# colmap/glomap

Hardware: NVIDIA H100
Metric: observations/sec per BA LM-iteration (higher is better)
Workload: dtype f64

## Files before the change

glomap_b200/csrc/ba_kernels_v2.cuh:

```cuda
#pragma once
#include "ba_kernels.cuh"
#include "pcg.cuh"

namespace b200 {

struct BAViewV2 {
  const double* Ap;
  double* z4;
  const double* pts4;
  double* Ufk = nullptr;
  const IntrVarRec* ivar = nullptr;
  int C = 0;
};

template <int NK>
__device__ __forceinline__ void obs_intr_jac(const ObsCore& o, const Intr& in, const IntrVarRec& iv,
                                             double Jk[2][NK > 0 ? NK : 1]) {
#pragma unroll
  for (int j = 0; j < NK; ++j) {
    double jx = 0.0, jy = 0.0;
    if (j < iv.mb) intr_param_jac(in, iv.pidx[j], o.uv[0], o.uv[1], 1.0, jx, jy);
    if (!o.valid) jx = jy = 0.0;
    Jk[0][j] = jx;
    Jk[1][j] = jy;
  }
}
template <int NK>
__device__ __forceinline__ void obs_intr_rows(const ObsCore& o, const Intr& in, const IntrVarRec& iv,
                                              const double Jp[6], double Jk[2][NK > 0 ? NK : 1],
                                              double B[NK > 0 ? 3 * NK : 1]) {
  obs_intr_jac<NK>(o, in, iv, Jk);
#pragma unroll
  for (int j = 0; j < NK; ++j)
#pragma unroll
    for (int c = 0; c < 3; ++c) B[3 * j + c] = o.rho1 * (Jp[c] * Jk[0][j] + Jp[3 + c] * Jk[1][j]);
}

struct SegRec {
  double R[9];
  double4 t4;
  Intr in;
  const double* sr;
};
__device__ __forceinline__ void seg_records(const BAView& v, int seg, int cam, const double* __restrict__ cam_rec,
                                            const double* __restrict__ intr_rec, SegRec& s) {
  const double4 q4 = ld_rec32(cam_rec + (size_t)cam * kCamRec);
  s.t4 = ld_rec32(cam_rec + (size_t)cam * kCamRec + 4);
  s.in = ld_intr(intr_rec + (size_t)v.seg_intr[seg] * kIntrRec);
  s.sr = sensor_of_seg(v, seg);
  const double q[4] = {q4.x, q4.y, q4.z, q4.w};
  quat_to_R(q, s.R);
}
__device__ __forceinline__ void to_sensor(const double* __restrict__ sr, double x[3]) {
  if (!sr) return;
  const double x0 = x[0], x1 = x[1], x2 = x[2];
#pragma unroll
  for (int k = 0; k < 3; ++k) x[k] = sr[3 * k] * x0 + sr[3 * k + 1] * x1 + sr[3 * k + 2] * x2;
}
__device__ __forceinline__ void cam_frame_jac(const ObsCore& o, const double r[3], double a[2], double w[3]) {
  const ProjJac& p = o.pj;
  const double t0 = r[0] - p.u * r[2], t1 = r[1] - p.v * r[2];
  const double c = o.rho1 * p.iz;
  a[0] = c * (p.m00 * t0 + p.m01 * t1);
  a[1] = c * (p.m10 * t0 + p.m11 * t1);
  const double s0 = p.iz * (p.m00 * a[0] + p.m10 * a[1]), s1 = p.iz * (p.m01 * a[0] + p.m11 * a[1]);
  w[0] = s0;
  w[1] = s1;
  w[2] = -(p.u * s0 + p.v * s1);
}
__device__ __forceinline__ void rig_to_frame(const double* __restrict__ sr, double x[3]) {
  const double x0 = x[0], x1 = x[1], x2 = x[2];
#pragma unroll
  for (int k = 0; k < 3; ++k) x[k] = sr[k] * x0 + sr[3 + k] * x1 + sr[6 + k] * x2;
}
// ... 38 lines not shown
    p[i] = pv[k];
    yw[i] = 0.0;
  }
  if (c >= n_pack) return;
  const double* r = cam_rec + (size_t)c * kCamRec;
  const double q[4] = {r[0], r[1], r[2], r[3]};
  double R[9];
  quat_to_R(q, R);
  double* o = xp + (size_t)c * kXqStride;
#pragma unroll
  for (int k = 0; k < 3; ++k) {
    o[k] = R[k] * pv[0] + R[3 + k] * pv[1] + R[6 + k] * pv[2];
    o[3 + k] = R[k] * pv[3] + R[3 + k] * pv[4] + R[6 + k] * pv[5];
  }
}

__global__ void ba2_pad_points(int P, const double* __restrict__ points, double* __restrict__ pts4) {
  const int p = blockIdx.x * blockDim.x + threadIdx.x;
  if (p >= P) return;
  const double x = points[3 * (size_t)p], y = points[3 * (size_t)p + 1], z = points[3 * (size_t)p + 2];
  st_rec32(pts4 + 4 * (size_t)p, x, y, z, 0.0);
}

template <int NK>
__global__ void __launch_bounds__(128, NK > 0 ? 3 : B200_LC_MIN_CTAS) ba2_linearize_cams(BAView v, BAViewV2 v2, const double* __restrict__ cam_rec,
                                                         const double* __restrict__ intr_rec, double huber_a) {
  const int warp = (blockIdx.x * blockDim.x + threadIdx.x) >> 5;
  const int lane = threadIdx.x & 31;
  if (warp >= v.n_segs) return;
  const int cam = v.seg_cam[warp];
  const int b = v.seg_begin[warp], e = v.seg_end[warp];
  SegRec sg;
  seg_records(v, warp, cam, cam_rec, intr_rec, sg);
  double U[21], g[6];
#pragma unroll
  for (int k = 0; k < 21; ++k) U[k] = 0.0;
#pragma unroll
  for (int k = 0; k < 6; ++k) g[k] = 0.0;
  const int cmask = (int)(__double_as_longlong(sg.t4.w) & 0xff);
  const bool tvar = !(cmask & 2), rvar = !(cmask & 1);
  constexpr int NKK = NK > 0 ? NK : 1;
  const int blk = v.seg_intr[warp];
  IntrVarRec iv{};
  if (NK > 0) iv = v2.ivar[blk];
  double Ukk[NKK * (NKK + 1) / 2], gk[NKK], Ufk[6][NKK];
#pragma unroll
  for (int k = 0; k < NKK * (NKK + 1) / 2; ++k) Ukk[k] = 0.0;
#pragma unroll
  for (int k = 0; k < NKK; ++k) {
    gk[k] = 0.0;
#pragma unroll
    for (int i2 = 0; i2 < 6; ++i2) Ufk[i2][k] = 0.0;
  }
  const double* __restrict__ pts4 = v2.pts4;
  int i = b + lane;
  int pt_nxt = 0;
  double2 xy = make_double2(0, 0);
  double4 Xc = make_double4(0, 0, 0, 0);
  if (i < e) {
    const int pt0 = ld_stream(v.pt_c + i);
    if (i + 32 < e) pt_nxt = ld_stream(v.pt_c + i + 32);
    xy = ld_stream(v.xy_c + i);
    Xc = ld_rec32(pts4 + 4 * (size_t)pt0);
  }
  for (; i < e; i += 32) {
    double4 Xn = Xc;
    double2 xyn = xy;
    int pt_nn = 0;
    if (i + 32 < e) {
      Xn = ld_rec32(pts4 + 4 * (size_t)pt_nxt);
      xyn = ld_stream(v.xy_c + i + 32);
    }
    if (i + 64 < e) pt_nn = ld_stream(v.pt_c + i + 64);
    const double X0 = Xc.x, X1 = Xc.y, X2 = Xc.z;
    ObsCore o;
    obs_core_R(sg.R, sg.t4, sg.in, sg.sr, X0, X1, X2, xy, huber_a, o);
    double Jc[2][6];
#pragma unroll
    for (int a = 0; a < 2; ++a) {
      const double j0 = o.J[3 * a], j1 = o.J[3 * a + 1], j2 = o.J[3 * a + 2];
      Jc[a][0] = rvar ? -2.0 * (j1 * o.RX[2] - j2 * o.RX[1]) : 0.0;
      Jc[a][1] = rvar ? -2.0 * (j2 * o.RX[0] - j0 * o.RX[2]) : 0.0;
      Jc[a][2] = rvar ? -2.0 * (j0 * o.RX[1] - j1 * o.RX[0]) : 0.0;
      Jc[a][3] = tvar ? j0 : 0.0;
      Jc[a][4] = tvar ? j1 : 0.0;
      Jc[a][5] = tvar ? j2 : 0.0;
    }
    const double e0 = o.rho1 * o.e[0], e1 = o.rho1 * o.e[1];
    int idx = 0;
#pragma unroll
    for (int i2 = 0; i2 < 6; ++i2) {
      const double s0 = o.rho1 * Jc[0][i2], s1 = o.rho1 * Jc[1][i2];
#pragma unroll
      for (int j = i2; j < 6; ++j) U[idx++] += s0 * Jc[0][j] + s1 * Jc[1][j];
      g[i2] += Jc[0][i2] * e0 + Jc[1][i2] * e1;
    }
    if (NK > 0) {
      double Jk[2][NKK];
      obs_intr_jac<NK>(o, sg.in, iv, Jk);
      int ik = 0;
#pragma unroll
      for (int a = 0; a < NK; ++a) {
        const double s0 = o.rho1 * Jk[0][a], s1 = o.rho1 * Jk[1][a];
#pragma unroll
        for (int c = a; c < NK; ++c) Ukk[ik++] += s0 * Jk[0][c] + s1 * Jk[1][c];
        gk[a] += Jk[0][a] * e0 + Jk[1][a] * e1;
#pragma unroll
        for (int i2 = 0; i2 < 6; ++i2) Ufk[i2][a] += Jc[0][i2] * s0 + Jc[1][i2] * s1;
      }
    }
    Xc = Xn; xy = xyn; pt_nxt = pt_nn;
  }
  if (NK > 0) {
    const size_t kb = (size_t)(v2.C + blk);
    int ik = 0;
#pragma unroll
    for (int a = 0; a < NK; ++a) {
#pragma unroll
      for (int c = a; c < NK; ++c) {
        const double sacc = warp_sum(Ukk[ik++]);
        if (lane == 0 && sacc != 0.0) atomicAdd(&v.U[kb * 21 + sym_idx(6, a, c)], sacc);
      }
      const double sg = warp_sum(gk[a]);
      if (lane == 0 && sg != 0.0) atomicAdd(&v.gc[kb * 6 + a], sg);
#pragma unroll
      for (int i2 = 0; i2 < 6; ++i2) {
        const double sf = warp_sum(Ufk[i2][a]);
        if (lane == 0 && sf != 0.0) atomicAdd(&v2.Ufk[((size_t)cam * 6 + i2) * NK + a], sf);
      }
    }
  }
#pragma unroll
  for (int k = 0; k < 21; ++k) {
    const double s = warp_sum(U[k]);
    if (lane == k && s != 0.0) atomicAdd(&v.U[(size_t)cam * 21 + k], s);
  }
#pragma unroll
  for (int k = 0; k < 6; ++k) {
    const double s = warp_sum(g[k]);
    if (lane == 21 + k && s != 0.0) atomicAdd(&v.gc[(size_t)cam * 6 + k], s);
  }
}

__global__ void __launch_bounds__(128, B200_SD_MIN_CTAS) ba2_schur_diag(BAView v, BAViewV2 v2, const double* __restrict__ cam_rec,
                                                                        const double* __restrict__ intr_rec, double huber_a) {
  const int warp = (blockIdx.x * blockDim.x + threadIdx.x) >> 5;
  const int lane = threadIdx.x & 31;
  if (warp >= v.n_segs) return;
  const int cam = v.seg_cam[warp];
  const int b = v.seg_begin[warp], e = v.seg_end[warp];
  SegRec sg;
  seg_records(v, warp, cam, cam_rec, intr_rec, sg);
  double RR[6] = {0, 0, 0, 0, 0, 0}, RT[9] = {0, 0, 0, 0, 0, 0, 0, 0, 0}, TT[6] = {0, 0, 0, 0, 0, 0};
  int i = b + lane;
  int pt_nxt = 0;
  double2 xy = make_double2(0, 0), va = xy, vb = xy, vc = xy;
  double4 Xc = make_double4(0, 0, 0, 0);
  if (i < e) {
    const int pt0 = ld_stream(v.pt_c + i);
    if (i + 32 < e) pt_nxt = ld_stream(v.pt_c + i + 32);
    xy = ld_stream(v.xy_c + i);
    Xc = ld_rec32(v2.pts4 + 4 * (size_t)pt0);
    const double2* vp = reinterpret_cast<const double2*>(v.Vinv + (size_t)pt0 * 6);
    va = vp[0]; vb = vp[1]; vc = vp[2];
  }
  for (; i < e; i += 32) {
    double4 Xn = Xc;
    double2 xyn = xy, van = va, vbn = vb, vcn = vc;
    int pt_nn = 0;
    if (i + 32 < e) {
      Xn = ld_rec32(v2.pts4 + 4 * (size_t)pt_nxt);
      xyn = ld_stream(v.xy_c + i + 32);
      const double2* vp = reinterpret_cast<const double2*>(v.Vinv + (size_t)pt_nxt * 6);
      van = vp[0]; vbn = vp[1]; vcn = vp[2];
    }
    if (i + 64 < e) pt_nn = ld_stream(v.pt_c + i + 64);
    ObsCore o;
    obs_core_R(sg.R, sg.t4, sg.in, sg.sr, Xc.x, Xc.y, Xc.z, xy, huber_a, o);
    double X[3] = {o.RX[0], o.RX[1], o.RX[2]};
    to_sensor(sg.sr, X);
    const ProjJac& pj = o.pj;
    const double vi[6] = {va.x, va.y, vb.x, vb.y, vc.x, vc.y};
    double e0[3] = {1.0, 0.0, -pj.u}, e1[3] = {0.0, 1.0, -pj.v};
    if (sg.sr) {
#pragma unroll
      for (int c = 0; c < 3; ++c) {
        e0[c] = sg.sr[c] - pj.u * sg.sr[6 + c];
        e1[c] = sg.sr[3 + c] - pj.v * sg.sr[6 + c];
      }
    }
    double l0[3], l1[3], t0[3], t1[3];
#pragma unroll
    for (int c = 0; c < 3; ++c) {
      l0[c] = e0[0] * sg.R[c] + e0[1] * sg.R[3 + c] + e0[2] * sg.R[6 + c];
      l1[c] = e1[0] * sg.R[c] + e1[1] * sg.R[3 + c] + e1[2] * sg.R[6 + c];
    }
    sym3_mul(vi, l0, t0);
    sym3_mul(vi, l1, t1);
    const double q00 = l0[0] * t0[0] + l0[1] * t0[1] + l0[2] * t0[2];
    const double q01 = l0[0] * t1[0] + l0[1] * t1[1] + l0[2] * t1[2];
    const double q11 = l1[0] * t1[0] + l1[1] * t1[1] + l1[2] * t1[2];
    const double k00 = pj.m00 * pj.m00 + pj.m10 * pj.m10, k01 = pj.m00 * pj.m01 + pj.m10 * pj.m11,
                 k11 = pj.m01 * pj.m01 + pj.m11 * pj.m11;
    const double a00 = k00 * q00 + k01 * q01, a01 = k00 * q01 + k01 * q11;
    const double a10 = k01 * q00 + k11 * q01, a11 = k01 * q01 + k11 * q11;
    const double sc = o.rho1 * pj.iz * pj.iz, c2 = sc * sc;
    const double h00 = c2 * (a00 * k00 + a01 * k01), h01 = c2 * (a00 * k01 + a01 * k11), h11 = c2 * (a10 * k01 + a11 * k11);
    double N[3][3];
    N[0][0] = h00; N[0][1] = N[1][0] = h01; N[1][1] = h11;
    N[0][2] = N[2][0] = -(h00 * pj.u + h01 * pj.v);
    N[1][2] = N[2][1] = -(h01 * pj.u + h11 * pj.v);
    N[2][2] = -(N[0][2] * pj.u + N[1][2] * pj.v);
    double P[3][3];
#pragma unroll
    for (int c = 0; c < 3; ++c) {
      const double n0 = N[0][c], n1 = N[1][c], n2 = N[2][c];
      P[0][c] = 2.0 * (X[1] * n2 - X[2] * n1);
      P[1][c] = 2.0 * (X[2] * n0 - X[0] * n2);
// ... 2 lines not shown
    double PK[3][3];
#pragma unroll
    for (int r = 0; r < 3; ++r) {
      PK[r][0] = P[r][1] * X[2] - P[r][2] * X[1];
      PK[r][1] = -P[r][0] * X[2] + P[r][2] * X[0];
      PK[r][2] = P[r][0] * X[1] - P[r][1] * X[0];
    }
    RR[0] += -2.0 * PK[0][0]; RR[1] += -2.0 * PK[0][1]; RR[2] += -2.0 * PK[0][2];
    RR[3] += -2.0 * PK[1][1]; RR[4] += -2.0 * PK[1][2]; RR[5] += -2.0 * PK[2][2];
#pragma unroll
    for (int r = 0; r < 3; ++r)
#pragma unroll
      for (int c = 0; c < 3; ++c) RT[3 * r + c] += P[r][c];
    TT[0] += N[0][0]; TT[1] += N[0][1]; TT[2] += N[0][2]; TT[3] += N[1][1]; TT[4] += N[1][2]; TT[5] += N[2][2];
    Xc = Xn; xy = xyn; va = van; vb = vbn; vc = vcn; pt_nxt = pt_nn;
  }
#pragma unroll
  for (int k = 0; k < 6; ++k) RR[k] = warp_sum(RR[k]);
#pragma unroll
  for (int k = 0; k < 9; ++k) RT[k] = warp_sum(RT[k]);
#pragma unroll
  for (int k = 0; k < 6; ++k) TT[k] = warp_sum(TT[k]);
  if (lane == 0) {
    const int mask = (int)(__double_as_longlong(sg.t4.w) & 0xff);
    double R[9] = {1, 0, 0, 0, 1, 0, 0, 0, 1};
    if (sg.sr) {
      for (int r = 0; r < 3; ++r)
        for (int c = 0; c < 3; ++c) R[3 * r + c] = sg.sr[3 * c + r];
    }
    double M[6][6];
    const double rr[3][3] = {{RR[0], RR[1], RR[2]}, {RR[1], RR[3], RR[4]}, {RR[2], RR[4], RR[5]}};
    const double tt[3][3] = {{TT[0], TT[1], TT[2]}, {TT[1], TT[3], TT[4]}, {TT[2], TT[4], TT[5]}};
    for (int r = 0; r < 3; ++r)
      for (int c = 0; c < 3; ++c) {
        M[r][c] = rr[r][c];
        M[3 + r][3 + c] = tt[r][c];
        M[r][3 + c] = RT[3 * r + c];
        M[3 + c][r] = RT[3 * r + c];
      }
    double T[6][6];
    for (int blk = 0; blk < 2; ++blk)
      for (int r = 0; r < 3; ++r)
        for (int c = 0; c < 6; ++c)
          T[3 * blk + r][c] = R[3 * r] * M[3 * blk][c] + R[3 * r + 1] * M[3 * blk + 1][c] + R[3 * r + 2] * M[3 * blk + 2][c];
    int idx = 0;
    for (int r = 0; r < 6; ++r)
      for (int c = r; c < 6; ++c, ++idx) {
        const int cb = c / 3, cc = c % 3;
        double s = T[r][3 * cb] * R[3 * cc] + T[r][3 * cb + 1] * R[3 * cc + 1] + T[r][3 * cb + 2] * R[3 * cc + 2];
        const bool rfix = (r < 3) ? (mask & 1) : (mask & 2), cfix = (c < 3) ? (mask & 1) : (mask & 2);
        if (rfix || cfix) s = 0.0;
// ... 168 lines not shown
  a0 = block_sum(a0, scratch);
  a1 = block_sum(a1, scratch);
  a2 = block_sum(a2, scratch);
  a3 = block_sum(a3, scratch);
  if (threadIdx.x == 0) {
    double* o = out + 4 * (size_t)blockIdx.x;
    o[0] = a0; o[1] = a1; o[2] = a2; o[3] = a3;
  }
}

__global__ void ba2_point_rhs_z(BAView v, BAViewV2 v2) {
  const int p = blockIdx.x * blockDim.x + threadIdx.x;
  if (p >= v.P) return;
  double vi[6], g[3], z[3];
#pragma unroll
  for (int k = 0; k < 6; ++k) vi[k] = v.Vinv[6 * (size_t)p + k];
#pragma unroll
  for (int k = 0; k < 3; ++k) g[k] = v.gp[3 * (size_t)p + k];
  sym3_mul(vi, g, z);
  const bool pvalid = (int)(v.pt_begin[p + 1] - v.pt_begin[p]) >= v.min_views;
  *reinterpret_cast<double4*>(v2.z4 + 4 * (size_t)p) = pvalid ? make_double4(z[0], z[1], z[2], 0.0) : make_double4(0, 0, 0, 0);
}

template <int NK>
__global__ void __launch_bounds__(128, B200_PB_MIN_CTAS) ba2_pass_b(BAView v, BAViewV2 v2, const double* __restrict__ cam_rec,
                                                 const double* __restrict__ intr_rec, double huber_a,
                                                 double* __restrict__ y, const PcgCtl* __restrict__ ctl, int seg_lo,
                                                 int seg_hi) {
  if (ctl && ctl->done) return;
  const int warp = seg_lo + ((blockIdx.x * blockDim.x + threadIdx.x) >> 5);
  const int lane = threadIdx.x & 31;
  if (warp >= seg_hi) return;
  const int cam = v.seg_cam[warp];
  const int b = v.seg_begin[warp], e = v.seg_end[warp];
  const int blk = v.seg_intr[warp];
  SegRec sg;
  seg_records(v, warp, cam, cam_rec, intr_rec, sg);
  constexpr int NKK = NK > 0 ? NK : 1;
  IntrVarRec iv{};
  if (NK > 0) iv = v2.ivar[blk];
  double acc[6] = {0, 0, 0, 0, 0, 0};
  double accK[NKK];
#pragma unroll
  for (int k = 0; k < NKK; ++k) accK[k] = 0.0;
  const uint64_t keep = l2_policy_evict_last();
  int i = b + lane;
  int pt_nxt = 0;
  double4 X = make_double4(0, 0, 0, 0), z = X;
  double2 xy = make_double2(0, 0);
  if (i < e) {
    const int pt0 = ld_stream(v.pt_c + i);
    if (i + 32 < e) pt_nxt = ld_stream(v.pt_c + i + 32);
    X = ld_rec32(v2.pts4 + 4 * (size_t)pt0);
    z = ld_keep4(v2.z4 + 4 * (size_t)pt0, keep);
    xy = ld_stream(v.xy_c + i);
  }
  for (; i < e; i += 32) {
    double4 Xn = X, zn = z;
    double2 xyn = xy;
    int pt_nn = 0;
    if (i + 32 < e) {
      Xn = ld_rec32(v2.pts4 + 4 * (size_t)pt_nxt);
      zn = ld_keep4(v2.z4 + 4 * (size_t)pt_nxt, keep);
      xyn = ld_stream(v.xy_c + i + 32);
    }
    if (i + 64 < e) pt_nn = ld_stream(v.pt_c + i + 64);
    ObsCore o;
    obs_core_R(sg.R, sg.t4, sg.in, sg.sr, X.x, X.y, X.z, xy, huber_a, o);
    double P[3] = {o.RX[0], o.RX[1], o.RX[2]};
    to_sensor(sg.sr, P);
    double r[3] = {sg.R[0] * z.x + sg.R[1] * z.y + sg.R[2] * z.z,
                   sg.R[3] * z.x + sg.R[4] * z.y + sg.R[5] * z.z,
                   sg.R[6] * z.x + sg.R[7] * z.y + sg.R[8] * z.z};
    to_sensor(sg.sr, r);
    double a[2], w[3];
    cam_frame_jac(o, r, a, w);
    acc[0] += P[1] * w[2] - P[2] * w[1];
    acc[1] += P[2] * w[0] - P[0] * w[2];
    acc[2] += P[0] * w[1] - P[1] * w[0];
    acc[3] += w[0];
    acc[4] += w[1];
    acc[5] += w[2];
    if (NK > 0) {
      double Jk[2][NKK];
      obs_intr_jac<NK>(o, sg.in, iv, Jk);
#pragma unroll
      for (int k = 0; k < NK; ++k) accK[k] += Jk[0][k] * a[0] + Jk[1][k] * a[1];
    }
    X = Xn; z = zn; xy = xyn; pt_nxt = pt_nn;
  }
#pragma unroll
  for (int k = 0; k < 6; ++k) acc[k] = warp_sum(acc[k]);
  if (sg.sr) {
    rig_to_frame(sg.sr, acc);
    rig_to_frame(sg.sr, acc + 3);
  }
  const int mask = (int)(__double_as_longlong(sg.t4.w) & 0xff);
#pragma unroll
  for (int k = 0; k < 6; ++k) {
    const double s = k < 3 ? 2.0 * acc[k] : acc[k];
    const bool fixed = k < 3 ? (mask & 1) : (mask & 2);
    if (lane == k && !fixed && s != 0.0) atomicAdd(&y[(size_t)cam * 6 + k], -s);
  }
  if (NK > 0) {
    const size_t kb = (size_t)(v2.C + blk);
#pragma unroll
    for (int k = 0; k < NK; ++k) {
      const double sk = warp_sum(accK[k]);
      if (lane == 0 && sk != 0.0) atomicAdd(&y[kb * 6 + k], -sk);
    }
  }
}

__global__ void ba2k_pack_xk(int C, const double* __restrict__ cam_rec, const double* __restrict__ x, double* __restrict__ xp,
                             const PcgCtl* __restrict__ ctl) {
  if (ctl && ctl->done) return;
  const int c = blockIdx.x * blockDim.x + threadIdx.x;
  if (c >= C) return;
  const int blk = (int)(__double_as_longlong(cam_rec[(size_t)c * kCamRec + 7]) >> 8);
  xp[(size_t)c * kXqStride + 6] = x[(size_t)(C + blk) * 6];
// ... 54 lines not shown
```

glomap_b200/csrc/ba_solver.cuh:

```cuda
#pragma once
#include <cub/cub.cuh>

#include <algorithm>
#include <climits>
#include <cmath>
#include <cstdlib>
#include <vector>

#include "../../include/b200sfm_testing.h"
#include "ba_kernels.cuh"
#include "ba_kernels_v2.cuh"
#include "ba_kernels_v3.cuh"
#include "ba_kernels_ext.cuh"
#include "filter_kernels.cuh"
#include "processor_kernels.cuh"
#include "context.cuh"
#include "pcg.cuh"

namespace b200 {

constexpr double kSliceL2Share = 1.0 / 6.0;

__global__ void k_expand_obs_pt(int P, const unsigned* __restrict__ pt_begin, int* __restrict__ obs_pt) {
  const int p = blockIdx.x * blockDim.x + threadIdx.x;
// ... 125 lines not shown
  b200::ExtView ext_view() {
    b200::ExtView e;
    e.C = C; e.K = K; e.S = S; e.ivar = ivar.p; e.sensor_var = (ext_s && S > 0) ? sensor_var.p : nullptr;
    return e;
  }
  bool use_v2 = false;
  bool use_ell = false;
  int ell_groups = 0, ell_ctas = 0, ell_bpart_rows = 0;
  long long ell_rows = 0;
  DevBuf<int> ell_row0, ell_pt, ell_len, ell_slot, ell_cam;
  DevBuf<double2> ell_xy;
  DevBuf<unsigned short> ell_sensor;
  DevBuf<double> ell_A, ell_part;
  b200::EllView ell_view() {
    b200::EllView e;
    e.n_groups = ell_groups; e.row0 = ell_row0.p; e.pt = ell_pt.p; e.len = ell_len.p; e.cam = ell_cam.p; e.xy = ell_xy.p;
    e.sensor = S > 0 ? ell_sensor.p : nullptr; e.A = ell_A.p; e.B = kfast ? ell_B.p : nullptr;
    return e;
  }
  DevBuf<double> z4, pts4, xq, bpart, bpart2;
  size_t smem_k3v2 = 0;
  bool kfast = false;
  int nk = 0;
  DevBuf<double> ell_B, Ufk;
  b200::BAViewV2 view2() {
    b200::BAViewV2 w;
    w.Ap = W.p; w.z4 = z4.p; w.pts4 = pts4.p;
    w.Ufk = kfast ? Ufk.p : nullptr; w.ivar = ivar.p; w.C = C;
    return w;
  }
  int cur = 0;
  DevBuf<double> cam_rec, intr_rec;
  DevBuf<double> W, V, Vinv, gp, lin , Sd, Minv, jscale_c, jscale_p, Dc;
  DevBuf<double> px, pr, pz, pp, pq, yw, bvec;
  DevBuf<double> scal;
  b200::EventTimer timer_lin, timer_mv;
  size_t smem_k1 = 0, smem_k3 = 0;

  double* U() { return lin.p; }
  double* gc() { return lin.p + (size_t)CB * 21; }
  double* cost_ptr() { return lin.p + (size_t)CB * 27; }

  BAView view() {
    BAView v;
    v.C = C; v.P = P; v.K = K; v.N = N; v.n_tiles = n_tiles; v.n_segs = n_segs; v.min_views = min_views;
    v.obs_cam = obs_cam.p; v.obs_pt = obs_pt.p; v.obs_xy = obs_xy.p; v.pt_begin = pt_begin.p;
// ... 335 lines not shown
    }
    if (use_ell) {
      const int nwp = ell_ctas * (kEllThreads / 32);
#define B200_LIN_P(NKV)                                                                                                   \
  B200_LAUNCH(ctx, ba3_linearize_points<NKV>, ell_ctas, kEllThreads, 0, v, ell_view(), cam_rec.p, intr_rec.p, points[cur].p, \
              huber_a, points_var ? 1 : 0, ell_part.p, ell_part.p + nwp, ivar.p)
      if (kfast && nk == 2) B200_LIN_P(2);
      else if (kfast && nk == 1) B200_LIN_P(1);
      else B200_LIN_P(0);
#undef B200_LIN_P
      B200_LAUNCH(ctx, ba3_reduce_partials, 1, 1024, 0, nwp, ell_part.p, ell_part.p + nwp, scal.p, scal.p + 1);
    } else if (use_v2)
      B200_LAUNCH(ctx, ba_linearize_points<true>, n_tiles, kTile, smem_k1, v, cam_rec.p, intr_rec.p, points[cur].p, huber_a,
                  points_var ? 1 : 0, scal.p);
    else
      B200_LAUNCH(ctx, ba_linearize_points<false>, n_tiles, kTile, smem_k1, v, cam_rec.p, intr_rec.p, points[cur].p, huber_a,
                  points_var ? 1 : 0, scal.p);
    if (profile) B200_CUDA_OK(cudaEventRecord(e1, s));
    if (n_segs > 0) {
      const int sgrid = cdiv((long long)n_segs * 32, 128);
      if (kfast) {
        Ufk.zero(s);
        B200_LAUNCH(ctx, ba2_pad_points, cdiv(P, 256), 256, 0, P, points[cur].p, pts4.p);
        if (nk == 2) B200_LAUNCH(ctx, ba2_linearize_cams<2>, sgrid, 128, 0, v, view2(), cam_rec.p, intr_rec.p, huber_a);
        else B200_LAUNCH(ctx, ba2_linearize_cams<1>, sgrid, 128, 0, v, view2(), cam_rec.p, intr_rec.p, huber_a);
      } else if (ext) {
        B200_LAUNCH(ctx, bax_linearize_blocks<0>, sgrid, 128, 0, v, ext_view(), cam_rec.p, intr_rec.p, points[cur].p, huber_a);
        if (ext_k) B200_LAUNCH(ctx, bax_linearize_blocks<1>, sgrid, 128, 0, v, ext_view(), cam_rec.p, intr_rec.p, points[cur].p, huber_a);
        if (ext_s) B200_LAUNCH(ctx, bax_linearize_blocks<2>, sgrid, 128, 0, v, ext_view(), cam_rec.p, intr_rec.p, points[cur].p, huber_a);
      } else if (use_v2) {
        B200_LAUNCH(ctx, ba2_pad_points, cdiv(P, 256), 256, 0, P, points[cur].p, pts4.p);
        B200_LAUNCH(ctx, ba2_linearize_cams<0>, sgrid, 128, 0, v, view2(), cam_rec.p, intr_rec.p, huber_a);
      } else {
        B200_LAUNCH(ctx, ba_linearize_cams, sgrid, 128, 0, v, cam_rec.p, intr_rec.p, points[cur].p, huber_a);
      }
    }
    B200_CUDA_OK(cudaMemcpyAsync(cost_ptr(), scal.p, sizeof(double), cudaMemcpyDeviceToDevice, s));
    B200_CUDA_OK(cudaMemcpyAsync(cost_ptr() + 1 + ctx->rank, scal.p + 1, sizeof(double), cudaMemcpyDeviceToDevice, s));
    ctx->allreduce_sum(lin.p, (size_t)CB * 27 + 1 + (size_t)ctx->world);
    B200_CUDA_OK(cudaMemsetAsync(scal.p + 1, 0, sizeof(double), s));
    B200_LAUNCH(ctx, ba_finalize_cams, cdiv(nbk, 128), 128, 0, nbk, U(), gc(), cam_mask.p, jscale_c.p, first ? 1 : 0,
                scal.p, cost_ptr() + 1, ctx->world);
    B200_CUDA_OK(cudaMemcpyAsync(ctx->h_scal, cost_ptr(), sizeof(double), cudaMemcpyDeviceToHost, s));
    B200_CUDA_OK(cudaMemcpyAsync(ctx->h_scal + 1, scal.p + 1, sizeof(double), cudaMemcpyDeviceToHost, s));
    B200_CUDA_OK(cudaStreamSynchronize(s));
    cost = ctx->h_scal[0];
    gmax = ctx->h_scal[1];
  }

  DevBuf<double> bear_res;
  void undistort(double* h_out) {
    using namespace b200;
    cudaStream_t s = ctx->stream;
    if (bear_res.n < (size_t)N * 3) bear_res.alloc((size_t)std::max<long long>(N, 1) * 3);
    if (N > 0)
// ... 117 lines not shown
      if (ext_k && ext_s) B200_EXT_A(true, true);
      else if (ext_k) B200_EXT_A(true, false);
      else if (ext_s) B200_EXT_A(false, true);
      else B200_EXT_A(false, false);
#undef B200_EXT_A
    }
    if (n_segs > 0) {
#define B200_EXT_B(WK, WS)                                                                                              \
  B200_LAUNCH(ctx, (bax_pass_b<WK, WS>), sgrid, 128, 0, v, ex, view2(), cam_rec.p, intr_rec.p, points[cur].p, x, huber_a, y, ctl)
      if (ext_k && ext_s) B200_EXT_B(true, true);
      else if (ext_k) B200_EXT_B(true, false);
      else if (ext_s) B200_EXT_B(false, true);
      else B200_EXT_B(false, false);
#undef B200_EXT_B
    }
  }

  void launch_pass_b(const b200::BAView& v, double huber_a, double* y, const b200::PcgCtl* ctl, int seg_lo = 0,
                     int seg_hi = -1) {
    using namespace b200;
    if (seg_hi < 0) seg_hi = n_segs;
    if (seg_hi <= seg_lo) return;
    const int grid = cdiv((long long)(seg_hi - seg_lo) * 32, 128);
#define B200_PASS_B(NKV) \
  B200_LAUNCH(ctx, ba2_pass_b<NKV>, grid, 128, 0, v, view2(), cam_rec.p, intr_rec.p, huber_a, y, ctl, seg_lo, seg_hi)
    if (kfast && nk == 2) B200_PASS_B(2);
    else if (kfast) B200_PASS_B(1);
    else B200_PASS_B(0);
#undef B200_PASS_B
  }
  void launch_pass_a0(const b200::BAView& v, double radius, const b200::PcgCtl* ctl) {
    using namespace b200;
    if (kfast && nk == 2)
      B200_LAUNCH(ctx, (ba3_pass_a<0, 2>), ell_ctas, kEllThreads, 0, v, ell_view(), view2(), xq.p, points[cur].p, nullptr, radius, nullptr, ctl);
    else if (kfast)
      B200_LAUNCH(ctx, (ba3_pass_a<0, 1>), ell_ctas, kEllThreads, 0, v, ell_view(), view2(), xq.p, points[cur].p, nullptr, radius, nullptr, ctl);
    else
      B200_LAUNCH(ctx, (ba3_pass_a<0, 0>), ell_ctas, kEllThreads, 0, v, ell_view(), view2(), xq.p, points[cur].p, nullptr, radius, nullptr, ctl);
  }
  void launch_cross(const double* x, double* y, const b200::PcgCtl* ctl) {
    using namespace b200;
    if (nk == 2) B200_LAUNCH(ctx, ba2k_cross<2>, cdiv(C, 256), 256, 0, C, K, cam_rec.p, Ufk.p, x, y, ctl);
    else B200_LAUNCH(ctx, ba2k_cross<1>, cdiv(C, 256), 256, 0, C, K, cam_rec.p, Ufk.p, x, y, ctl);
  }

  bool matrix_free() const { return ext && !kfast; }
  bool schur_jacobi_on(const b200sfm_ba_opts& o, bool points_var) const {
    return points_var && o.preconditioner == 1 && !matrix_free();
  }

  void matvec(const double* x, double* y, const b200sfm_ba_opts& o, double radius, bool points_var, bool split_ar,
// ... 33 lines not shown
                  nullptr, 0, ctl);
    }
    if (profile) B200_CUDA_OK(cudaEventRecord(e1, s));
    if (split_ar) {
      ctx->allreduce_sum(y + (size_t)(C / 2) * 6, nB6 - (size_t)(C / 2) * 6);
      B200_CUDA_OK(cudaStreamWaitEvent(s, ctx->ev_comm, 0));
    } else {
      ctx->allreduce_sum(y, nB6);
    }
  }

  StepResult compute_step(const b200sfm_ba_opts& o, double radius, bool points_var, bool set_jscale_p, bool profile) {
    using namespace b200;
    cudaStream_t s = ctx->stream;
    BAView v = view();
    const int nB6 = nbk * 6;
    if (points_var) B200_LAUNCH(ctx, ba_damp_points, cdiv(P, 256), 256, 0, P, V.p, jscale_p.p, set_jscale_p ? 1 : 0, radius, Vinv.p);
    B200_LAUNCH(ctx, ba_damp_cams, cdiv(nB6, 256), 256, 0, nbk, U(), jscale_c.p, radius, Dc.p);
    const bool recomp = matrix_free();
    const bool schur_jacobi = schur_jacobi_on(o, points_var);
    double* yrhs = Sd.p + (size_t)CB * 21;
    Sd.zero(s);
    if (schur_jacobi && n_segs > 0) {
      if (use_v2)
        B200_LAUNCH(ctx, ba2_schur_diag, cdiv((long long)n_segs * 32, 128), 128, 0, v, view2(), cam_rec.p, intr_rec.p,
                    o.thres_loss_function);
      else B200_LAUNCH(ctx, ba_schur_diag, cdiv((long long)n_segs * 32, 128), 128, 0, v);
    }
    if (points_var) {
      if (use_v2) {
        B200_LAUNCH(ctx, ba2_point_rhs_z, cdiv(P, 256), 256, 0, v, view2());
        if (recomp) ext_matvec(nullptr, yrhs, o.thres_loss_function, radius, true, nullptr);
        else if (n_segs > 0) launch_pass_b(v, o.thres_loss_function, yrhs, nullptr);
      } else {
        B200_LAUNCH(ctx, ba_schur_pass<1>, n_tiles, kTile, smem_k3, v, nullptr, yrhs, nullptr, nullptr, radius, nullptr);
      }
    } else if (recomp) {
      z4.zero(s);
    }
    if (schur_jacobi || points_var) ctx->allreduce_sum(Sd.p, (size_t)CB * 27);
    B200_LAUNCH(ctx, ba_build_precond, cdiv(nbk, 128), 128, 0, nbk, U(), Dc.p, schur_jacobi ? Sd.p : nullptr, Minv.p);
    B200_LAUNCH(ctx, k_rhs, cdiv(nB6, 256), 256, 0, nB6, gc(), points_var ? yrhs : nullptr, bvec.p);
    const int max_it = std::max(1, o.pcg_max_iterations);
    const int nblk = cdiv(nbk, kPcgThreads);
    ctx->pcgh.ensure(max_it, (size_t)nblk * 3, ctx->world);
    double* part_pq = ctx->pcgh.d_part;
    double* part_rz = ctx->pcgh.d_part + nblk;
    double* part_rr = ctx->pcgh.d_part + 2 * (size_t)nblk;
    PcgCtl* ctl = ctx->pcgh.d_ctl;
    StepResult res;
// ... 111 lines not shown
          for (int j = 0; j < 3; ++j)
            if (nfoc[h_intr_model[k]][j] >= 0) idx.push_back(nfoc[h_intr_model[k]][j]);
        if (all_var) { idx.push_back(pp[h_intr_model[k]][0]); idx.push_back(pp[h_intr_model[k]][1]); }
        std::sort(idx.begin(), idx.end());
        h_ivar[k].col0 = 0;
        h_ivar[k].mb = (int)idx.size();
        for (size_t j = 0; j < idx.size(); ++j) h_ivar[k].pidx[j] = idx[j];
        ext_k = ext_k || !idx.empty();
      }
      B200_CUDA_OK(cudaMemcpyAsync(ivar.p, h_ivar.data(), K * sizeof(b200::IntrVarRec), cudaMemcpyHostToDevice, s));
    }
    ext_s = false;
    if (o.optimize_rig_poses && S > 0)
      for (int i = 0; i < S; ++i) ext_s = ext_s || h_sensor_var[i] != 0;
    ext = ext_k || ext_s;
    nbk = ext ? CB : C;
    B200_CUDA_OK(cudaStreamSynchronize(s));
    use_v2 = ext || (o.design != 1);
    use_ell = use_v2 && (ext || !(getenv("B200SFM_ELL") && atoi(getenv("B200SFM_ELL")) == 0));
    nk = 0;
    if (ext_k)
      for (int k = 0; k < K; ++k) nk = std::max(nk, h_ivar[k].mb);
    kfast = ext_k && !ext_s && S == 0 && nk <= 2 && !(getenv("B200SFM_KFAST") && atoi(getenv("B200SFM_KFAST")) == 0);
    if (kfast) {
      const size_t cells = (size_t)std::max<long long>(ell_rows, 1) * 32;
      if (ell_B.n < cells * 3 * nk) ell_B.alloc(cells * 3 * nk);
      if (Ufk.n < (size_t)C * 6 * nk) Ufk.alloc((size_t)C * 6 * nk);
    }
  }
  void launch_eff_mask(const b200sfm_ba_opts& o) {
    B200_LAUNCH(ctx, b200::k_eff_mask, b200::cdiv(C, 256), 256, 0, C, cam_mask_base.p, o.optimize_rotations ? 0 : 1,
                o.optimize_translation ? 0 : 1, cam_mask.p);
  }

  void reject_step() { build_records(cur); }

  int solve(const b200sfm_ba_opts& o, b200sfm_lm_stats* st) {
    using namespace b200;
    cudaStream_t s = ctx->stream;
    select_paths(o);
    const bool l2_persist = use_v2 && !(getenv("B200SFM_L2_PERSIST") && atoi(getenv("B200SFM_L2_PERSIST")) == 0) &&
                            l2_persist_window(s, ctx->device, z4.p, z4.bytes());
    const long long launches0 = ctx->launches;
    timer_lin.reset();
    timer_mv.reset();
    cudaEvent_t ev0, ev1;
// ... 159 lines not shown
```

glomap_b200/csrc/common.cuh:

```cuda
#pragma once
#include <cuda_runtime.h>
#include <stdint.h>
#include <stdio.h>

#include <string>

namespace b200 {

#ifndef B200_TILE
#define B200_TILE 128
#endif
#ifndef B200_K1_MIN_CTAS
#define B200_K1_MIN_CTAS 5
#endif
#ifndef B200_K3_MIN_CTAS
#define B200_K3_MIN_CTAS 8
#endif
#ifndef B200_PA_MIN_CTAS
#define B200_PA_MIN_CTAS 12
#endif
#ifndef B200_LC_MIN_CTAS
#define B200_LC_MIN_CTAS 3
#endif
#ifndef B200_PB_MIN_CTAS
#define B200_PB_MIN_CTAS 4
#endif
#ifndef B200_SD_MIN_CTAS
#define B200_SD_MIN_CTAS 3
#endif
#ifndef B200_E1_MIN_CTAS
#define B200_E1_MIN_CTAS 4
#endif
#ifndef B200_E1_PIPE
#define B200_E1_PIPE 1
#endif
#ifndef B200_EA_MIN_CTAS
#define B200_EA_MIN_CTAS 8
#endif
#ifndef B200_EA2_MIN_CTAS
#define B200_EA2_MIN_CTAS 6
#endif
#ifndef B200_STREAM_HINTS
#define B200_STREAM_HINTS 1
#endif
constexpr int kTile = B200_TILE;
constexpr int kTilePts = 64;
constexpr int kWDoubles = 18;
constexpr int kWBytes = kWDoubles * 8;

#define B200_CUDA_OK(expr)                                                                     \
  do {                                                                                         \
// ... 275 lines not shown
```

Baseline: 1.573 billion.

## Stage per-segment camera records in shared memory and specialize kernels on radial/rig

Per-segment camera rotation, translation, intrinsics and sensor transform move out of per-thread registers into a 256-byte shared-memory record per warp. Each observation reloads them with explicit ld.shared. The kernels gain compile-time RAD/RIG template flags, so the non-radial and non-rig variants drop the distortion and sensor-transform code, and the host picks the variant at launch. The point is to lower register pressure so more CTAs fit per SM, and minimum-CTA launch bounds go from 3 to 4 for the linearize and Schur-diagonal kernels. The cost is extra shared-memory loads in the inner loop and the risk of register spills under the tighter bounds.

```diff
diff --git a/glomap_b200/csrc/ba_kernels_v2.cuh b/glomap_b200/csrc/ba_kernels_v2.cuh
--- a/glomap_b200/csrc/ba_kernels_v2.cuh
+++ b/glomap_b200/csrc/ba_kernels_v2.cuh
@@ -36,20 +36,59 @@
     for (int c = 0; c < 3; ++c) B[3 * j + c] = o.rho1 * (Jp[c] * Jk[0][j] + Jp[3 + c] * Jk[1][j]);
 }
 
-struct SegRec {
+struct SegSmem {
+  double R[9], t[3];
+  double fx, fy, cx, cy, k1, k2, model;
+  double packed;
+  double sr[12];
+};
+static_assert(sizeof(SegSmem) == 32 * sizeof(double), "one 256-B record per warp");
+template <bool RIG>
+__device__ __forceinline__ void seg_fill(const BAView& v, int seg, int cam, const double* __restrict__ cam_rec,
+                                         const double* __restrict__ intr_rec, SegSmem& s) {
+  const double4 q4 = ld_rec32(cam_rec + (size_t)cam * kCamRec);
+  const double4 t4 = ld_rec32(cam_rec + (size_t)cam * kCamRec + 4);
+  const double q[4] = {q4.x, q4.y, q4.z, q4.w};
   double R[9];
-  double4 t4;
-  Intr in;
-  const double* sr;
-};
-__device__ __forceinline__ void seg_records(const BAView& v, int seg, int cam, const double* __restrict__ cam_rec,
-                                            const double* __restrict__ intr_rec, SegRec& s) {
-  const double4 q4 = ld_rec32(cam_rec + (size_t)cam * kCamRec);
-  s.t4 = ld_rec32(cam_rec + (size_t)cam * kCamRec + 4);
-  s.in = ld_intr(intr_rec + (size_t)v.seg_intr[seg] * kIntrRec);
-  s.sr = sensor_of_seg(v, seg);
-  const double q[4] = {q4.x, q4.y, q4.z, q4.w};
-  quat_to_R(q, s.R);
+  quat_to_R(q, R);
+#pragma unroll
+  for (int k = 0; k < 9; ++k) s.R[k] = R[k];
+  s.t[0] = t4.x; s.t[1] = t4.y; s.t[2] = t4.z;
+  s.packed = t4.w;
+  const double* ir = intr_rec + (size_t)v.seg_intr[seg] * kIntrRec;
+  s.fx = ir[0]; s.fy = ir[1]; s.cx = ir[2]; s.cy = ir[3]; s.k1 = ir[4]; s.k2 = ir[5]; s.model = ir[6];
+  if (RIG) {
+    const double* sr = v.sensor_rec + (size_t)v.seg_sensor[seg] * kSensorRec;
+#pragma unroll
+    for (int k = 0; k < 12; ++k) s.sr[k] = sr[k];
+  }
+}
+__device__ __forceinline__ double lds(const double* p) {
+  double x;
+  asm volatile("ld.shared.f64 %0, [%1];" : "=d"(x) : "r"((unsigned)__cvta_generic_to_shared(p)) : "memory");
+  return x;
+}
+__device__ __forceinline__ void seg_R(const SegSmem& s, double R[9]) {
+#pragma unroll
+  for (int k = 0; k < 9; ++k) R[k] = lds(&s.R[k]);
+}
+__device__ __forceinline__ double4 seg_t4(const SegSmem& s) { return make_double4(lds(&s.t[0]), lds(&s.t[1]), lds(&s.t[2]), 0.0); }
+template <int N>
+__device__ __forceinline__ void seg_sensor(const SegSmem& s, double sr[12]) {
+#pragma unroll
+  for (int k = 0; k < N; ++k) sr[k] = lds(&s.sr[k]);
+}
+template <int NK, bool RAD>
+__device__ __forceinline__ Intr seg_intr(const SegSmem& s) {
+  return Intr{lds(&s.fx), lds(&s.fy), lds(&s.cx), lds(&s.cy), RAD ? lds(&s.k1) : 0.0, RAD ? lds(&s.k2) : 0.0,
+              NK > 0 ? (int)lds(&s.model) : 0};
+}
+template <int NK, bool RAD, bool RIG>
+__device__ __forceinline__ void seg_obs_core(const SegSmem& s, const double R[9], double X0, double X1, double X2,
+                                             double2 xy, double huber_a, ObsCore& o) {
+  double sr[12];
+  if (RIG) seg_sensor<12>(s, sr);
+  obs_core_R(R, seg_t4(s), seg_intr<NK, RAD>(s), RIG ? sr : nullptr, X0, X1, X2, xy, huber_a, o);
 }
 __device__ __forceinline__ void to_sensor(const double* __restrict__ sr, double x[3]) {
   if (!sr) return;
@@ -134,22 +173,24 @@
   st_rec32(pts4 + 4 * (size_t)p, x, y, z, 0.0);
 }
 
-template <int NK>
-__global__ void __launch_bounds__(128, NK > 0 ? 3 : B200_LC_MIN_CTAS) ba2_linearize_cams(BAView v, BAViewV2 v2, const double* __restrict__ cam_rec,
+template <int NK, bool RAD, bool RIG>
+__global__ void __launch_bounds__(128, NK > 0 ? B200_LCK_MIN_CTAS : (RIG ? B200_RIG_MIN_CTAS : B200_LC_MIN_CTAS)) ba2_linearize_cams(BAView v, BAViewV2 v2, const double* __restrict__ cam_rec,
                                                          const double* __restrict__ intr_rec, double huber_a) {
+  __shared__ SegSmem seg_sm[4];
   const int warp = (blockIdx.x * blockDim.x + threadIdx.x) >> 5;
   const int lane = threadIdx.x & 31;
   if (warp >= v.n_segs) return;
   const int cam = v.seg_cam[warp];
   const int b = v.seg_begin[warp], e = v.seg_end[warp];
-  SegRec sg;
-  seg_records(v, warp, cam, cam_rec, intr_rec, sg);
+  if (lane == 0) seg_fill<RIG>(v, warp, cam, cam_rec, intr_rec, seg_sm[threadIdx.x >> 5]);
+  __syncwarp();
+  const SegSmem& sg = seg_sm[threadIdx.x >> 5];
   double U[21], g[6];
 #pragma unroll
   for (int k = 0; k < 21; ++k) U[k] = 0.0;
 #pragma unroll
   for (int k = 0; k < 6; ++k) g[k] = 0.0;
-  const int cmask = (int)(__double_as_longlong(sg.t4.w) & 0xff);
+  const int cmask = (int)(__double_as_longlong(lds(&sg.packed)) & 0xff);
   const bool tvar = !(cmask & 2), rvar = !(cmask & 1);
   constexpr int NKK = NK > 0 ? NK : 1;
   const int blk = v.seg_intr[warp];
@@ -186,7 +227,11 @@
     if (i + 64 < e) pt_nn = ld_stream(v.pt_c + i + 64);
     const double X0 = Xc.x, X1 = Xc.y, X2 = Xc.z;
     ObsCore o;
-    obs_core_R(sg.R, sg.t4, sg.in, sg.sr, X0, X1, X2, xy, huber_a, o);
+    {
+      double R[9];
+      seg_R(sg, R);
+      seg_obs_core<NK, RAD, RIG>(sg, R, X0, X1, X2, xy, huber_a, o);
+    }
     double Jc[2][6];
 #pragma unroll
     for (int a = 0; a < 2; ++a) {
@@ -209,7 +254,7 @@
     }
     if (NK > 0) {
       double Jk[2][NKK];
-      obs_intr_jac<NK>(o, sg.in, iv, Jk);
+      obs_intr_jac<NK>(o, seg_intr<NK, RAD>(sg), iv, Jk);
       int ik = 0;
 #pragma unroll
       for (int a = 0; a < NK; ++a) {
@@ -254,15 +299,18 @@
   }
 }
 
-__global__ void __launch_bounds__(128, B200_SD_MIN_CTAS) ba2_schur_diag(BAView v, BAViewV2 v2, const double* __restrict__ cam_rec,
+template <bool RAD, bool RIG>
+__global__ void __launch_bounds__(128, RIG ? B200_RIG_MIN_CTAS : B200_SD_MIN_CTAS) ba2_schur_diag(BAView v, BAViewV2 v2, const double* __restrict__ cam_rec,
                                                                         const double* __restrict__ intr_rec, double huber_a) {
+  __shared__ SegSmem seg_sm[4];
   const int warp = (blockIdx.x * blockDim.x + threadIdx.x) >> 5;
   const int lane = threadIdx.x & 31;
   if (warp >= v.n_segs) return;
   const int cam = v.seg_cam[warp];
   const int b = v.seg_begin[warp], e = v.seg_end[warp];
-  SegRec sg;
-  seg_records(v, warp, cam, cam_rec, intr_rec, sg);
+  if (lane == 0) seg_fill<RIG>(v, warp, cam, cam_rec, intr_rec, seg_sm[threadIdx.x >> 5]);
+  __syncwarp();
+  const SegSmem& sg = seg_sm[threadIdx.x >> 5];
   double RR[6] = {0, 0, 0, 0, 0, 0}, RT[9] = {0, 0, 0, 0, 0, 0, 0, 0, 0}, TT[6] = {0, 0, 0, 0, 0, 0};
   int i = b + lane;
   int pt_nxt = 0;
@@ -288,24 +336,34 @@
     }
     if (i + 64 < e) pt_nn = ld_stream(v.pt_c + i + 64);
     ObsCore o;
-    obs_core_R(sg.R, sg.t4, sg.in, sg.sr, Xc.x, Xc.y, Xc.z, xy, huber_a, o);
+    {
+      double R[9];
+      seg_R(sg, R);
+      seg_obs_core<0, RAD, RIG>(sg, R, Xc.x, Xc.y, Xc.z, xy, huber_a, o);
+    }
     double X[3] = {o.RX[0], o.RX[1], o.RX[2]};
-    to_sensor(sg.sr, X);
     const ProjJac& pj = o.pj;
     const double vi[6] = {va.x, va.y, vb.x, vb.y, vc.x, vc.y};
     double e0[3] = {1.0, 0.0, -pj.u}, e1[3] = {0.0, 1.0, -pj.v};
-    if (sg.sr) {
+    if (RIG) {
+      double sr[12];
+      seg_sensor<9>(sg, sr);
+      to_sensor(sr, X);
 #pragma unroll
       for (int c = 0; c < 3; ++c) {
-        e0[c] = sg.sr[c] - pj.u * sg.sr[6 + c];
-        e1[c] = sg.sr[3 + c] - pj.v * sg.sr[6 + c];
+        e0[c] = sr[c] - pj.u * sr[6 + c];
+        e1[c] = sr[3 + c] - pj.v * sr[6 + c];
       }
     }
     double l0[3], l1[3], t0[3], t1[3];
-#pragma unroll
-    for (int c = 0; c < 3; ++c) {
-      l0[c] = e0[0] * sg.R[c] + e0[1] * sg.R[3 + c] + e0[2] * sg.R[6 + c];
-      l1[c] = e1[0] * sg.R[c] + e1[1] * sg.R[3 + c] + e1[2] * sg.R[6 + c];
+    {
+      double R[9];
+      seg_R(sg, R);
+#pragma unroll
+      for (int c = 0; c < 3; ++c) {
+        l0[c] = e0[0] * R[c] + e0[1] * R[3 + c] + e0[2] * R[6 + c];
+        l1[c] = e1[0] * R[c] + e1[1] * R[3 + c] + e1[2] * R[6 + c];
+      }
     }
     sym3_mul(vi, l0, t0);
     sym3_mul(vi, l1, t1);
@@ -354,11 +412,11 @@
 #pragma unroll
   for (int k = 0; k < 6; ++k) TT[k] = warp_sum(TT[k]);
   if (lane == 0) {
-    const int mask = (int)(__double_as_longlong(sg.t4.w) & 0xff);
+    const int mask = (int)(__double_as_longlong(lds(&sg.packed)) & 0xff);
     double R[9] = {1, 0, 0, 0, 1, 0, 0, 0, 1};
-    if (sg.sr) {
+    if (RIG) {
       for (int r = 0; r < 3; ++r)
-        for (int c = 0; c < 3; ++c) R[3 * r + c] = sg.sr[3 * c + r];
+        for (int c = 0; c < 3; ++c) R[3 * r + c] = lds(&sg.sr[3 * c + r]);
     }
     double M[6][6];
     const double rr[3][3] = {{RR[0], RR[1], RR[2]}, {RR[1], RR[3], RR[4]}, {RR[2], RR[4], RR[5]}};
@@ -573,11 +631,12 @@
   *reinterpret_cast<double4*>(v2.z4 + 4 * (size_t)p) = pvalid ? make_double4(z[0], z[1], z[2], 0.0) : make_double4(0, 0, 0, 0);
 }
 
-template <int NK>
-__global__ void __launch_bounds__(128, B200_PB_MIN_CTAS) ba2_pass_b(BAView v, BAViewV2 v2, const double* __restrict__ cam_rec,
+template <int NK, bool RAD, bool RIG>
+__global__ void __launch_bounds__(128, NK > 0 ? B200_PBK_MIN_CTAS : B200_PB_MIN_CTAS) ba2_pass_b(BAView v, BAViewV2 v2, const double* __restrict__ cam_rec,
                                                  const double* __restrict__ intr_rec, double huber_a,
                                                  double* __restrict__ y, const PcgCtl* __restrict__ ctl, int seg_lo,
                                                  int seg_hi) {
+  __shared__ SegSmem seg_sm[4];
   if (ctl && ctl->done) return;
   const int warp = seg_lo + ((blockIdx.x * blockDim.x + threadIdx.x) >> 5);
   const int lane = threadIdx.x & 31;
@@ -585,8 +644,9 @@
   const int cam = v.seg_cam[warp];
   const int b = v.seg_begin[warp], e = v.seg_end[warp];
   const int blk = v.seg_intr[warp];
-  SegRec sg;
-  seg_records(v, warp, cam, cam_rec, intr_rec, sg);
+  if (lane == 0) seg_fill<RIG>(v, warp, cam, cam_rec, intr_rec, seg_sm[threadIdx.x >> 5]);
+  __syncwarp();
+  const SegSmem& sg = seg_sm[threadIdx.x >> 5];
   constexpr int NKK = NK > 0 ? NK : 1;
   IntrVarRec iv{};
   if (NK > 0) iv = v2.ivar[blk];
@@ -617,13 +677,22 @@
     }
     if (i + 64 < e) pt_nn = ld_stream(v.pt_c + i + 64);
     ObsCore o;
-    obs_core_R(sg.R, sg.t4, sg.in, sg.sr, X.x, X.y, X.z, xy, huber_a, o);
+    double r[3];
+    {
+      double R[9];
+      seg_R(sg, R);
+      r[0] = R[0] * z.x + R[1] * z.y + R[2] * z.z;
+      r[1] = R[3] * z.x + R[4] * z.y + R[5] * z.z;
+      r[2] = R[6] * z.x + R[7] * z.y + R[8] * z.z;
+      seg_obs_core<NK, RAD, RIG>(sg, R, X.x, X.y, X.z, xy, huber_a, o);
+    }
     double P[3] = {o.RX[0], o.RX[1], o.RX[2]};
-    to_sensor(sg.sr, P);
-    double r[3] = {sg.R[0] * z.x + sg.R[1] * z.y + sg.R[2] * z.z,
-                   sg.R[3] * z.x + sg.R[4] * z.y + sg.R[5] * z.z,
-                   sg.R[6] * z.x + sg.R[7] * z.y + sg.R[8] * z.z};
-    to_sensor(sg.sr, r);
+    if (RIG) {
+      double sr[12];
+      seg_sensor<9>(sg, sr);
+      to_sensor(sr, P);
+      to_sensor(sr, r);
+    }
     double a[2], w[3];
     cam_frame_jac(o, r, a, w);
     acc[0] += P[1] * w[2] - P[2] * w[1];
@@ -634,7 +703,7 @@
     acc[5] += w[2];
     if (NK > 0) {
       double Jk[2][NKK];
-      obs_intr_jac<NK>(o, sg.in, iv, Jk);
+      obs_intr_jac<NK>(o, seg_intr<NK, RAD>(sg), iv, Jk);
 #pragma unroll
       for (int k = 0; k < NK; ++k) accK[k] += Jk[0][k] * a[0] + Jk[1][k] * a[1];
     }
@@ -642,11 +711,13 @@
   }
 #pragma unroll
   for (int k = 0; k < 6; ++k) acc[k] = warp_sum(acc[k]);
-  if (sg.sr) {
-    rig_to_frame(sg.sr, acc);
-    rig_to_frame(sg.sr, acc + 3);
-  }
-  const int mask = (int)(__double_as_longlong(sg.t4.w) & 0xff);
+  if (RIG) {
+    double sr[12];
+    seg_sensor<9>(sg, sr);
+    rig_to_frame(sr, acc);
+    rig_to_frame(sr, acc + 3);
+  }
+  const int mask = (int)(__double_as_longlong(lds(&sg.packed)) & 0xff);
 #pragma unroll
   for (int k = 0; k < 6; ++k) {
     const double s = k < 3 ? 2.0 * acc[k] : acc[k];
diff --git a/glomap_b200/csrc/ba_solver.cuh b/glomap_b200/csrc/ba_solver.cuh
--- a/glomap_b200/csrc/ba_solver.cuh
+++ b/glomap_b200/csrc/ba_solver.cuh
@@ -171,6 +171,7 @@
   size_t smem_k3v2 = 0;
   bool kfast = false;
   int nk = 0;
+  bool radial = false;
   DevBuf<double> ell_B, Ufk;
   b200::BAViewV2 view2() {
     b200::BAViewV2 w;
@@ -552,15 +553,22 @@
       if (kfast) {
         Ufk.zero(s);
         B200_LAUNCH(ctx, ba2_pad_points, cdiv(P, 256), 256, 0, P, points[cur].p, pts4.p);
-        if (nk == 2) B200_LAUNCH(ctx, ba2_linearize_cams<2>, sgrid, 128, 0, v, view2(), cam_rec.p, intr_rec.p, huber_a);
-        else B200_LAUNCH(ctx, ba2_linearize_cams<1>, sgrid, 128, 0, v, view2(), cam_rec.p, intr_rec.p, huber_a);
+#define B200_LIN_C(NKV, RAD, RIG) \
+  B200_LAUNCH(ctx, (ba2_linearize_cams<NKV, RAD, RIG>), sgrid, 128, 0, v, view2(), cam_rec.p, intr_rec.p, huber_a)
+        if (nk == 2 && radial) B200_LIN_C(2, true, false);
+        else if (nk == 2) B200_LIN_C(2, false, false);
+        else B200_LIN_C(1, false, false);
       } else if (ext) {
         B200_LAUNCH(ctx, bax_linearize_blocks<0>, sgrid, 128, 0, v, ext_view(), cam_rec.p, intr_rec.p, points[cur].p, huber_a);
         if (ext_k) B200_LAUNCH(ctx, bax_linearize_blocks<1>, sgrid, 128, 0, v, ext_view(), cam_rec.p, intr_rec.p, points[cur].p, huber_a);
         if (ext_s) B200_LAUNCH(ctx, bax_linearize_blocks<2>, sgrid, 128, 0, v, ext_view(), cam_rec.p, intr_rec.p, points[cur].p, huber_a);
       } else if (use_v2) {
         B200_LAUNCH(ctx, ba2_pad_points, cdiv(P, 256), 256, 0, P, points[cur].p, pts4.p);
-        B200_LAUNCH(ctx, ba2_linearize_cams<0>, sgrid, 128, 0, v, view2(), cam_rec.p, intr_rec.p, huber_a);
+        if (S > 0 && radial) B200_LIN_C(0, true, true);
+        else if (S > 0) B200_LIN_C(0, false, true);
+        else if (radial) B200_LIN_C(0, true, false);
+        else B200_LIN_C(0, false, false);
+#undef B200_LIN_C
       } else {
         B200_LAUNCH(ctx, ba_linearize_cams, sgrid, 128, 0, v, cam_rec.p, intr_rec.p, points[cur].p, huber_a);
       }
@@ -724,11 +732,15 @@
     if (seg_hi < 0) seg_hi = n_segs;
     if (seg_hi <= seg_lo) return;
     const int grid = cdiv((long long)(seg_hi - seg_lo) * 32, 128);
-#define B200_PASS_B(NKV) \
-  B200_LAUNCH(ctx, ba2_pass_b<NKV>, grid, 128, 0, v, view2(), cam_rec.p, intr_rec.p, huber_a, y, ctl, seg_lo, seg_hi)
-    if (kfast && nk == 2) B200_PASS_B(2);
-    else if (kfast) B200_PASS_B(1);
-    else B200_PASS_B(0);
+#define B200_PASS_B(NKV, RAD, RIG) \
+  B200_LAUNCH(ctx, (ba2_pass_b<NKV, RAD, RIG>), grid, 128, 0, v, view2(), cam_rec.p, intr_rec.p, huber_a, y, ctl, seg_lo, seg_hi)
+    if (kfast && nk == 2 && radial) B200_PASS_B(2, true, false);
+    else if (kfast && nk == 2) B200_PASS_B(2, false, false);
+    else if (kfast) B200_PASS_B(1, false, false);
+    else if (S > 0 && radial) B200_PASS_B(0, true, true);
+    else if (S > 0) B200_PASS_B(0, false, true);
+    else if (radial) B200_PASS_B(0, true, false);
+    else B200_PASS_B(0, false, false);
 #undef B200_PASS_B
   }
   void launch_pass_a0(const b200::BAView& v, double radius, const b200::PcgCtl* ctl) {
@@ -808,10 +820,16 @@
     double* yrhs = Sd.p + (size_t)CB * 21;
     Sd.zero(s);
     if (schur_jacobi && n_segs > 0) {
-      if (use_v2)
-        B200_LAUNCH(ctx, ba2_schur_diag, cdiv((long long)n_segs * 32, 128), 128, 0, v, view2(), cam_rec.p, intr_rec.p,
-                    o.thres_loss_function);
-      else B200_LAUNCH(ctx, ba_schur_diag, cdiv((long long)n_segs * 32, 128), 128, 0, v);
+      if (use_v2) {
+#define B200_SCHUR_D(RAD, RIG)                                                                                   \
+  B200_LAUNCH(ctx, (ba2_schur_diag<RAD, RIG>), cdiv((long long)n_segs * 32, 128), 128, 0, v, view2(), cam_rec.p, \
+              intr_rec.p, o.thres_loss_function)
+        if (S > 0 && radial) B200_SCHUR_D(true, true);
+        else if (S > 0) B200_SCHUR_D(false, true);
+        else if (radial) B200_SCHUR_D(true, false);
+        else B200_SCHUR_D(false, false);
+#undef B200_SCHUR_D
+      } else B200_LAUNCH(ctx, ba_schur_diag, cdiv((long long)n_segs * 32, 128), 128, 0, v);
     }
     if (points_var) {
       if (use_v2) {
@@ -969,6 +987,7 @@
     if (ext_k)
       for (int k = 0; k < K; ++k) nk = std::max(nk, h_ivar[k].mb);
     kfast = ext_k && !ext_s && S == 0 && nk <= 2 && !(getenv("B200SFM_KFAST") && atoi(getenv("B200SFM_KFAST")) == 0);
+    radial = std::any_of(h_intr_model.begin(), h_intr_model.end(), [](int m) { return m >= 2; });
     if (kfast) {
       const size_t cells = (size_t)std::max<long long>(ell_rows, 1) * 32;
       if (ell_B.n < cells * 3 * nk) ell_B.alloc(cells * 3 * nk);
diff --git a/glomap_b200/csrc/common.cuh b/glomap_b200/csrc/common.cuh
--- a/glomap_b200/csrc/common.cuh
+++ b/glomap_b200/csrc/common.cuh
@@ -20,13 +20,22 @@
 #define B200_PA_MIN_CTAS 12
 #endif
 #ifndef B200_LC_MIN_CTAS
-#define B200_LC_MIN_CTAS 3
+#define B200_LC_MIN_CTAS 4
+#endif
+#ifndef B200_LCK_MIN_CTAS
+#define B200_LCK_MIN_CTAS 3
 #endif
 #ifndef B200_PB_MIN_CTAS
 #define B200_PB_MIN_CTAS 4
 #endif
+#ifndef B200_PBK_MIN_CTAS
+#define B200_PBK_MIN_CTAS 4
+#endif
 #ifndef B200_SD_MIN_CTAS
-#define B200_SD_MIN_CTAS 3
+#define B200_SD_MIN_CTAS 4
+#endif
+#ifndef B200_RIG_MIN_CTAS
+#define B200_RIG_MIN_CTAS 3
 #endif
 #ifndef B200_E1_MIN_CTAS
 #define B200_E1_MIN_CTAS 4
```

New measurement: 1.608 billion (median of 6 runs). 2.2% higher.
